# lorenlugosch/end-to-end-SLU

Measured on AMD Instinct MI355X. Metric: utterances/sec (train step, 3 s @16 kHz, B=64), higher is better.
Workload: dtype f32 (trainable stages: exact fp32 MFMA; convolutions and GRU contractions of FROZEN stages: bf16x3 = every fp32 operand split EXACTLY into 3 bf16 terms (3 x 8 = 24 significand bits, fp32's exponent range), 6 bf16 MFMA products per fp32 product (only terms below 2^-24 |a b| dropped), fp32 accumulatio; 1 GPU; experiments/no_unfreezing.cfg SLU train step (frozen SincNet/conv/biGRU encoder in train mode + intent biGRU trained): fwd + 3-slot CE + bwd + grad all-reduce + Adam; batch_per_gpu=64, global_batch=64, samples_per_utterance=48000, parallelism=dp1, encoder_lookahead_batches=20

## Files before the change

end-to-end-slu_amd/csrc/slu_api.hip:

```cpp
#include "slu_common.h"
#include <string.h>

namespace slu {
static thread_local char g_err[512] = "";
void set_error(const char* fmt, ...) {
  va_list ap;
  va_start(ap, fmt);
  vsnprintf(g_err, sizeof(g_err), fmt, ap);
  va_end(ap);
}
}

extern "C" int slu_version(void) { return SLU_ABI_VERSION; }

extern "C" const char* slu_last_error(void) { return slu::g_err; }

extern "C" const char* slu_device_arch(void) {
  static thread_local char arch[256];
  arch[0] = 0;
  int dev = 0;
  hipDeviceProp_t prop;
  if (hipGetDevice(&dev) != hipSuccess) return arch;
  if (hipGetDeviceProperties(&prop, dev) != hipSuccess) return arch;
  strncpy(arch, prop.gcnArchName, sizeof(arch) - 1);
  arch[sizeof(arch) - 1] = 0;
  return arch;
}

extern "C" int slu_device_check(void) {
  const char* a = slu_device_arch();
  if (strncmp(a, "gfx950", 6) != 0)
    SLU_FAIL(SLU_ERR_DEVICE, "libslu_hip is built for gfx950 (MI355X) only; current device is '%s'", a);
  return SLU_OK;
}

extern "C" int slu_stream_create_cu_range(int64_t first_cu, int64_t n_cus, void** stream_out) {
  SLU_REQUIRE(stream_out, "slu_stream_create_cu_range: null pointer");
  int dev = 0;
  hipDeviceProp_t prop;
  if (hipGetDevice(&dev) != hipSuccess || hipGetDeviceProperties(&prop, dev) != hipSuccess)
    SLU_FAIL(SLU_ERR_DEVICE, "slu_stream_create_cu_range: no HIP device");
  const int64_t total = prop.multiProcessorCount;
  SLU_REQUIRE(first_cu >= 0 && n_cus > 0 && first_cu + n_cus <= total,
              "slu_stream_create_cu_range: range [%lld, %lld) outside the %lld CUs of the device",
              (long long)first_cu, (long long)(first_cu + n_cus), (long long)total);
  uint32_t mask[32] = {0};
  SLU_REQUIRE(total <= 32 * 32, "slu_stream_create_cu_range: device too large");
  for (int64_t i = first_cu; i < first_cu + n_cus; ++i) mask[i >> 5] |= 1u << (i & 31);
  hipStream_t st = nullptr;
  const hipError_t e = hipExtStreamCreateWithCUMask(&st, (uint32_t)((total + 31) / 32), mask);
  if (e != hipSuccess) SLU_FAIL(SLU_ERR_HIP, "hipExtStreamCreateWithCUMask: %s", hipGetErrorString(e));
  *stream_out = (void*)st;
  return SLU_OK;
}

namespace slu {
struct StageSeg { const unsigned char* src; unsigned char* dst; long long rows, row_bytes, src_stride; };
struct StageArgs { StageSeg seg[4]; int nseg; long long* set_ptr; long long set_value; };

__global__ void __launch_bounds__(256)
stage_inputs_kernel(const StageArgs a) {
  if (blockIdx.x == 0 && threadIdx.x == 0 && a.set_ptr) *a.set_ptr = a.set_value;
  for (int k = 0; k < a.nseg; ++k) {
    const StageSeg sg = a.seg[k];
    const bool vec = ((sg.row_bytes | sg.src_stride | (long long)(uintptr_t)sg.src | (long long)(uintptr_t)sg.dst) & 15) == 0;
    if (vec) {
      const long long per_row = sg.row_bytes >> 4, total = sg.rows * per_row;
      for (long long i = (long long)blockIdx.x * 256 + threadIdx.x; i < total; i += (long long)gridDim.x * 256) {
        const long long r = i / per_row, c = i - r * per_row;
        reinterpret_cast<uint4*>(sg.dst + r * sg.row_bytes)[c] = reinterpret_cast<const uint4*>(sg.src + r * sg.src_stride)[c];
      }
    } else {
      const long long total = sg.rows * sg.row_bytes;
      for (long long i = (long long)blockIdx.x * 256 + threadIdx.x; i < total; i += (long long)gridDim.x * 256) {
        const long long r = i / sg.row_bytes, c = i - r * sg.row_bytes;
        sg.dst[r * sg.row_bytes + c] = sg.src[r * sg.src_stride + c];
      }
    }
  }
}
}

namespace slu {
struct StoreArgs { unsigned long long v[64]; unsigned long long* dst; int n; };
__global__ void store_u64_kernel(const StoreArgs a) {
  if ((int)threadIdx.x < a.n) a.dst[threadIdx.x] = a.v[threadIdx.x];
}
}

extern "C" int slu_store_u64(uint64_t* dst, const uint64_t* values, int64_t count, void* stream) {
  SLU_REQUIRE(dst && values && count >= 1 && count <= 64, "slu_store_u64: 1..64 values");
  slu::StoreArgs a;
  for (int k = 0; k < (int)count; ++k) a.v[k] = values[k];
  a.dst = (unsigned long long*)dst; a.n = (int)count;
  hipLaunchKernelGGL(slu::store_u64_kernel, dim3(1), dim3(64), 0, (hipStream_t)stream, a);
  SLU_CHECK_LAUNCH("store_u64_kernel");
  return SLU_OK;
}

extern "C" int slu_stage_inputs(const void* const* src, void* const* dst, const int64_t* rows, const int64_t* row_bytes,
                                const int64_t* src_stride_bytes, int64_t count, int64_t* set_ptr, int64_t set_value,
                                void* stream) {
  SLU_REQUIRE(count >= 0 && count <= 4, "slu_stage_inputs: at most 4 segments");
  slu::StageArgs a;
  long long bytes = 0;
  for (int k = 0; k < (int)count; ++k) {
    SLU_REQUIRE(src[k] && dst[k] && rows[k] > 0 && row_bytes[k] > 0, "slu_stage_inputs: bad segment %d", k);
    a.seg[k].src = (const unsigned char*)src[k]; a.seg[k].dst = (unsigned char*)dst[k];
    a.seg[k].rows = rows[k]; a.seg[k].row_bytes = row_bytes[k]; a.seg[k].src_stride = src_stride_bytes[k];
    bytes += rows[k] * row_bytes[k];
  }
  a.nseg = (int)count; a.set_ptr = (long long*)set_ptr; a.set_value = set_value;
  long long blocks = (bytes / 16 + 255) / 256;
  if (blocks < 1) blocks = 1;
  if (blocks > 512) blocks = 512;
  hipLaunchKernelGGL(slu::stage_inputs_kernel, dim3((unsigned)blocks), dim3(256), 0, (hipStream_t)stream, a);
  SLU_CHECK_LAUNCH("stage_inputs_kernel");
  return SLU_OK;
}

namespace slu {
constexpr int MULTI_MAX = 32;
struct MultiArgs { const unsigned char* src[MULTI_MAX]; unsigned char* dst[MULTI_MAX]; long long bytes[MULTI_MAX]; int n; };

__global__ void __launch_bounds__(256)
copy_multi_kernel(const MultiArgs a) {
  const int k = blockIdx.y;
  if (k >= a.n) return;
  const unsigned char* __restrict__ s = a.src[k];
  unsigned char* __restrict__ d = a.dst[k];
  const long long nb = a.bytes[k];
  const bool vec = (((long long)(uintptr_t)s | (long long)(uintptr_t)d | nb) & 15) == 0;
  if (vec) {
    for (long long i = (long long)blockIdx.x * 256 + threadIdx.x; i < (nb >> 4); i += (long long)gridDim.x * 256)
      reinterpret_cast<uint4*>(d)[i] = reinterpret_cast<const uint4*>(s)[i];
  } else {
    for (long long i = (long long)blockIdx.x * 256 + threadIdx.x; i < (nb >> 2); i += (long long)gridDim.x * 256)
      reinterpret_cast<unsigned*>(d)[i] = reinterpret_cast<const unsigned*>(s)[i];
  }
}

struct ScaleArgs { float* ptr[MULTI_MAX]; long long numel[MULTI_MAX]; int n; const float* g; };

__global__ void __launch_bounds__(256)
scale_multi_kernel(const ScaleArgs a) {
  const int k = blockIdx.y;
  if (k >= a.n) return;
  const float g = a.g[0];
  float* __restrict__ p = a.ptr[k];
  for (long long i = (long long)blockIdx.x * 256 + threadIdx.x; i < a.numel[k]; i += (long long)gridDim.x * 256) p[i] *= g;
}
}

extern "C" int slu_multi_max(void) { return slu::MULTI_MAX; }

extern "C" int slu_copy_multi(const void* const* src, void* const* dst, const int64_t* nbytes, int64_t count, void* stream) {
  SLU_REQUIRE(src && dst && nbytes && count >= 1 && count <= slu::MULTI_MAX, "slu_copy_multi: 1..%d segments", slu::MULTI_MAX);
  slu::MultiArgs a;
  long long most = 0;
  for (int k = 0; k < (int)count; ++k) {
    SLU_REQUIRE(src[k] && dst[k] && nbytes[k] > 0 && nbytes[k] % 4 == 0 && (((uintptr_t)src[k] | (uintptr_t)dst[k]) & 3) == 0,
                "slu_copy_multi: segment %d must be a non-empty, 4-byte aligned run of whole words", k);
    a.src[k] = (const unsigned char*)src[k]; a.dst[k] = (unsigned char*)dst[k]; a.bytes[k] = nbytes[k];
    if (nbytes[k] > most) most = nbytes[k];
  }
  a.n = (int)count;
  long long bx = (most / 16 + 255) / 256;
  if (bx < 1) bx = 1;
  if (bx > 64) bx = 64;
  hipLaunchKernelGGL(slu::copy_multi_kernel, dim3((unsigned)bx, (unsigned)count), dim3(256), 0, (hipStream_t)stream, a);
  SLU_CHECK_LAUNCH("copy_multi_kernel");
  return SLU_OK;
}

extern "C" int slu_scale_multi(float* const* ptrs, const int64_t* numel, int64_t count, const float* scale_dev, void* stream) {
  SLU_REQUIRE(ptrs && numel && scale_dev && count >= 1 && count <= slu::MULTI_MAX, "slu_scale_multi: 1..%d tensors", slu::MULTI_MAX);
  slu::ScaleArgs a;
  long long most = 0;
  for (int k = 0; k < (int)count; ++k) {
    SLU_REQUIRE(ptrs[k] && numel[k] > 0, "slu_scale_multi: bad tensor %d", k);
    a.ptr[k] = ptrs[k]; a.numel[k] = numel[k];
    if (numel[k] > most) most = numel[k];
  }
  a.n = (int)count; a.g = scale_dev;
  long long bx = (most + 1023) / 1024;
  if (bx < 1) bx = 1;
  if (bx > 256) bx = 256;
  hipLaunchKernelGGL(slu::scale_multi_kernel, dim3((unsigned)bx, (unsigned)count), dim3(256), 0, (hipStream_t)stream, a);
  SLU_CHECK_LAUNCH("scale_multi_kernel");
  return SLU_OK;
}

namespace slu {
struct AbsmaxArgs { const float* ptr[MULTI_MAX]; long long numel[MULTI_MAX]; int n; unsigned* words; };

__global__ void __launch_bounds__(256)
absmax_multi_kernel(const AbsmaxArgs a) {
  const int k = blockIdx.y;
  if (k >= a.n) return;
  const float* __restrict__ p = a.ptr[k];
  unsigned mx = 0;
  for (long long i = (long long)blockIdx.x * 256 + threadIdx.x; i < a.numel[k]; i += (long long)gridDim.x * 256)
    mx = max(mx, __float_as_uint(p[i]) & 0x7fffffffu);
#pragma unroll
  for (int d = 32; d >= 1; d >>= 1) mx = max(mx, (unsigned)__shfl_xor((int)mx, d, 64));
  if ((threadIdx.x & 63) == 0 && mx > 0) atomicMax(a.words + k, mx);
// ... 37 lines not shown
```

end-to-end-slu_amd/csrc/slu_common.h:

```cpp
#pragma once
#include <hip/hip_runtime.h>
#include <stdint.h>
#include <stdio.h>
#include <stdarg.h>
#include "../../include/slu_hip.h"

namespace slu {

void set_error(const char* fmt, ...);

#define SLU_FAIL(code, ...)            \
  do {                                 \
    ::slu::set_error(__VA_ARGS__);     \
    return (code);                     \
  } while (0)

#define SLU_REQUIRE(cond, ...)                          \
  do {                                                  \
    if (!(cond)) SLU_FAIL(SLU_ERR_INVALID_ARG, __VA_ARGS__); \
  } while (0)

#define SLU_CHECK_LAUNCH(name)                                                        \
  do {                                                                                \
    hipError_t e__ = hipGetLastError();                                               \
    if (e__ != hipSuccess) SLU_FAIL(SLU_ERR_HIP, "%s: %s", name, hipGetErrorString(e__)); \
  } while (0)

static inline int64_t cdiv(int64_t a, int64_t b) { return (a + b - 1) / b; }

typedef float f32x4 __attribute__((ext_vector_type(4)));

__device__ __forceinline__ f32x4 mfma16(float a, float b, f32x4 c) {
  return __builtin_amdgcn_mfma_f32_16x16x4f32(a, b, c, 0, 0, 0);
}

__device__ __forceinline__ float sigmoidf_acc(float x) { return 1.0f / (1.0f + expf(-x)); }

}
```

end-to-end-slu_amd/csrc/slu_gemm_bf16.hip:

```cpp
#include "slu_bf16.h"

#include <cstdlib>

namespace slu {

constexpr int GB_BM = 128, GB_BN = 64, GB_THREADS = 256;

struct GemmBfParams {
  const unsigned short* A;
  long long a_plane, lda;
  const uint4* wp;
  const float* bias;
  float* C; long long ldc;
  int M, N, KC;
};

template <int NS>
__global__ void __launch_bounds__(256)
gemm_bf_pack_kernel(const float* __restrict__ W, long long ldw, long long w_cs, uint4* __restrict__ wp, int N, int K, int KC, int NT) {
  const int idx = blockIdx.x * blockDim.x + threadIdx.x;
  if (idx >= KC * NT * 64) return;
  const int lane = idx & 63, nt = (idx >> 6) % NT, kc = (idx >> 6) / NT;
  const int n = nt * 16 + (lane & 15), k0 = kc * 32 + (lane >> 4) * 8;
  unsigned short h[NS][8];
// ... 107 lines not shown
    const int kn = min((kc_) + 1, p.KC - 1);                                                         \
               \
    uint4 fa[NS][4];                                                                                 \
    _Pragma("unroll") for (int pl = 0; pl < NS; ++pl) _Pragma("unroll") for (int a = 0; a < 4; ++a)  \
      fa[pl][a] = sA[buf * STAGE_U4 + pl * GB_BM * 4 + a_frag[a]];                                   \
    __builtin_amdgcn_sched_barrier(0);                                                               \
    GB_DMA_A(kn, 1 - buf) GB_FETCH_B(kn, nxt)                                                        \
    __builtin_amdgcn_sched_barrier(0);             \
    _Pragma("unroll") for (int q = 0; q < SP::NPAIR; ++q) {                                          \
      _Pragma("unroll") for (int a = 0; a < 4; ++a) _Pragma("unroll") for (int b = 0; b < 2; ++b)    \
        accs[SP::ACC(q)][a][b] = mfma_split<NS>(fa[SP::PA(q)][a], cur[SP::PB(q)][b], accs[SP::ACC(q)][a][b]); \
    }                                                                                                \
    __builtin_amdgcn_sched_barrier(0);        \
    __syncthreads();              \
  }
  GB_DMA_A(0, 0)
  GB_FETCH_B(0, rb0)
  __syncthreads();
  for (int kc = 0; kc < p.KC; kc += 2) {
    GB_STEP(kc, 0, rb0, rb1)
    if (kc + 1 < p.KC) GB_STEP(kc + 1, 1, rb1, rb0)
  }
#undef GB_STEP
#undef GB_FETCH_B
#undef GB_DMA_A
  f32x4 acc[4][2];
#pragma unroll
  for (int a = 0; a < 4; ++a)
#pragma unroll
    for (int b = 0; b < 2; ++b) acc[a][b] = split_result<NS>(accs[0][a][b], accs[SP::NACC - 1][a][b]);

  float* const sC = reinterpret_cast<float*>(smem) + wave * (32 * 36);
  const int col4 = (lane & 7) * 4;
  float4 bv = make_float4(0.f, 0.f, 0.f, 0.f);
  const int ncol = n0 + wn * 32 + col4;
  if (p.bias) { bv.x = p.bias[ncol]; bv.y = p.bias[ncol + 1]; bv.z = p.bias[ncol + 2]; bv.w = p.bias[ncol + 3]; }
#pragma unroll
  for (int h = 0; h < 2; ++h) {
#pragma unroll
    for (int a2 = 0; a2 < 2; ++a2)
#pragma unroll
      for (int b = 0; b < 2; ++b)
#pragma unroll
        for (int r = 0; r < 4; ++r) sC[(a2 * 16 + 4 * kg + r) * 36 + b * 16 + i] = acc[2 * h + a2][b][r];
#pragma unroll
    for (int it = 0; it < 4; ++it) {
      const int rl = (lane >> 3) + 8 * it;
      const int m = m0 + wm * 64 + h * 32 + rl;
      const float4 v = *reinterpret_cast<const float4*>(&sC[rl * 36 + col4]);
      if (m < p.M)
        *reinterpret_cast<float4*>(p.C + (size_t)m * p.ldc + ncol) = make_float4(v.x + bv.x, v.y + bv.y, v.z + bv.z, v.w + bv.w);
    }
  }
}


template <int NS, int KC>
__global__ void __launch_bounds__(GB_THREADS, 2)
gemm_bf_panel_kernel(const GemmBfParams p) {
  constexpr int STAGE_U4 = NS * GB_BM * 4;
  constexpr int EPI_FLOATS = 4 * 32 * 36;
  __shared__ __attribute__((aligned(16))) char smem[KC * STAGE_U4 * 16 + EPI_FLOATS * 4];
  uint4* const sA = reinterpret_cast<uint4*>(smem);
  const int tid = threadIdx.x, lane = tid & 63;
  const int wave = __builtin_amdgcn_readfirstlane(tid >> 6);
  const int wm = wave >> 1, wn = wave & 1;
  const int i = lane & 15, kg = lane >> 4;
  const int NT = p.N / 16, NJ = p.N / GB_BN;
  const int m0 = blockIdx.x * GB_BM;
  typedef const __attribute__((address_space(1))) void* gptr_t;
  typedef __attribute__((address_space(3))) void* lptr_t;
  {
    const int srow = tid >> 2, sslot = tid & 3;
#pragma unroll
    for (int h = 0; h < 2; ++h) {
      const int r = srow + 64 * h, m = m0 + r;
      const unsigned short* src = p.A + (size_t)(m < p.M ? m : 0) * p.lda + swz_slot(r, sslot) * 8;
#pragma unroll
      for (int kc = 0; kc < KC; ++kc)
#pragma unroll
        for (int pl = 0; pl < NS; ++pl)
          __builtin_amdgcn_global_load_lds((gptr_t)(src + (size_t)pl * p.a_plane + kc * 32),
                                           (lptr_t)(sA + kc * STAGE_U4 + (pl * GB_BM + 64 * h + 16 * wave) * 4), 16, 0, 0);
    }
  }
  const uint4* b_src = p.wp + (size_t)(wn * 2) * 64 + lane;
  const size_t b_plane = (size_t)p.KC * NT * 64, b_chunk = (size_t)NT * 64;
  int a_frag[4];
#pragma unroll
  for (int a = 0; a < 4; ++a) {
    const int r = wm * 64 + a * 16 + i;
    a_frag[a] = r * 4 + swz_slot(r, kg);
  }
  const int col4 = (lane & 7) * 4;
  float* const sC = reinterpret_cast<float*>(smem + KC * STAGE_U4 * 16) + wave * (32 * 36);
  typedef Split<NS> SP;
  uint4 rb0[KC][NS][2], rb1[KC][NS][2];
  float4 bias0 = make_float4(0.f, 0.f, 0.f, 0.f), bias1 = bias0;
#define GP_FETCH(j_, dst, bdst)                                                                         \
  {                                                                                                     \
    const int jj = min((j_), NJ - 1);                                                                   \
    _Pragma("unroll") for (int kc = 0; kc < KC; ++kc) _Pragma("unroll") for (int pl = 0; pl < NS; ++pl) \
      _Pragma("unroll") for (int b = 0; b < 2; ++b)                                                     \
        dst[kc][pl][b] = b_src[(size_t)pl * b_plane + (size_t)kc * b_chunk + (size_t)(jj * 4 + b) * 64]; \
    if (p.bias) bdst = *reinterpret_cast<const float4*>(p.bias + jj * GB_BN + wn * 32 + col4);          \
  }
#define GP_TILE(j_, cur, bcur, nxt, bnxt)                                                               \
  {                                                                                                     \
    GP_FETCH((j_) + 1, nxt, bnxt)                                                                       \
    __builtin_amdgcn_sched_barrier(0);    \
    f32x4 accs[SP::NACC][4][2];                                                                         \
    _Pragma("unroll") for (int c = 0; c < SP::NACC; ++c)                                                \
      _Pragma("unroll") for (int a = 0; a < 4; ++a) _Pragma("unroll") for (int b = 0; b < 2; ++b)       \
        accs[c][a][b] = f32x4{0.f, 0.f, 0.f, 0.f};                                                      \
    _Pragma("unroll") for (int kc = 0; kc < KC; ++kc) {                                                 \
      uint4 fa[NS][4];                                                                                  \
      _Pragma("unroll") for (int pl = 0; pl < NS; ++pl) _Pragma("unroll") for (int a = 0; a < 4; ++a)   \
        fa[pl][a] = sA[kc * STAGE_U4 + pl * GB_BM * 4 + a_frag[a]];                                     \
      _Pragma("unroll") for (int q = 0; q < SP::NPAIR; ++q) {                                           \
        _Pragma("unroll") for (int a = 0; a < 4; ++a) _Pragma("unroll") for (int b = 0; b < 2; ++b)     \
          accs[SP::ACC(q)][a][b] = mfma_split<NS>(fa[SP::PA(q)][a], cur[kc][SP::PB(q)][b], accs[SP::ACC(q)][a][b]); \
      }                                                                                                 \
    }                                                                                                   \
    f32x4 acc[4][2];                                                                                    \
    _Pragma("unroll") for (int a = 0; a < 4; ++a) _Pragma("unroll") for (int b = 0; b < 2; ++b)         \
      acc[a][b] = split_result<NS>(accs[0][a][b], accs[SP::NACC - 1][a][b]);                            \
    const int ncol = (j_) * GB_BN + wn * 32 + col4;                                                     \
    _Pragma("unroll") for (int h = 0; h < 2; ++h) {                                                     \
      _Pragma("unroll") for (int a2 = 0; a2 < 2; ++a2) _Pragma("unroll") for (int b = 0; b < 2; ++b)    \
        _Pragma("unroll") for (int r = 0; r < 4; ++r)                                                   \
          sC[(a2 * 16 + 4 * kg + r) * 36 + b * 16 + i] = acc[2 * h + a2][b][r];                         \
      _Pragma("unroll") for (int it = 0; it < 4; ++it) {                                                \
        const int rl = (lane >> 3) + 8 * it;                                                            \
        const int m = m0 + wm * 64 + h * 32 + rl;                                                       \
        const float4 v = *reinterpret_cast<const float4*>(&sC[rl * 36 + col4]);                         \
        if (m < p.M)                                                                                    \
          *reinterpret_cast<float4*>(p.C + (size_t)m * p.ldc + ncol) =                                  \
              make_float4(v.x + bcur.x, v.y + bcur.y, v.z + bcur.z, v.w + bcur.w);                      \
      }                                                                                                 \
    }                                                                                                   \
  }
  GP_FETCH(0, rb0, bias0)
  __syncthreads();
  for (int j = 0; j < NJ; j += 2) {
    GP_TILE(j, rb0, bias0, rb1, bias1)
    if (j + 1 < NJ) GP_TILE(j + 1, rb1, bias1, rb0, bias0)
  }
#undef GP_TILE
#undef GP_FETCH
}


constexpr int GP_ROWS = 96;
constexpr int64_t GP_PANEL_MIN_M = 16 * 1024;

template <int NS, int KC>
__global__ void __launch_bounds__(GB_THREADS, 1)
gemm_bf_panel96_kernel(const GemmBfParams p) {
  constexpr int CH_U4 = NS * GP_ROWS * 4;
  typedef Split<NS> SP;
  extern __shared__ __attribute__((aligned(16))) char dsmem[];
  uint4* const sA = reinterpret_cast<uint4*>(dsmem);
  const int tid = threadIdx.x, lane = tid & 63;
  const int wave = __builtin_amdgcn_readfirstlane(tid >> 6);
  const int wm = wave >> 1, wn = wave & 1;
  const int i = lane & 15, kg = lane >> 4;
  const int NT = p.N / 16, NJ = p.N / GB_BN;
  const int m0 = blockIdx.x * GP_ROWS;
  typedef const __attribute__((address_space(1))) void* gptr_t;
  typedef __attribute__((address_space(3))) void* lptr_t;
  {
    const int rrow = lane >> 2, rslot = lane & 3;
    for (int u = wave; u < KC * NS * (GP_ROWS / 16); u += 4) {
      const int rg = u % (GP_ROWS / 16), pl = (u / (GP_ROWS / 16)) % NS, kc = u / ((GP_ROWS / 16) * NS);
      const int r = rg * 16 + rrow, m = m0 + r;
      const unsigned short* src = p.A + (size_t)pl * p.a_plane + (size_t)(m < p.M ? m : 0) * p.lda + kc * 32 + swz_slot(r, rslot) * 8;
      __builtin_amdgcn_global_load_lds((gptr_t)src, (lptr_t)(sA + kc * CH_U4 + (pl * GP_ROWS + rg * 16) * 4), 16, 0, 0);
    }
  }
  const uint4* b_src = p.wp + (size_t)(wn * 2) * 64 + lane;
  const size_t b_plane = (size_t)p.KC * NT * 64, b_chunk = (size_t)NT * 64;
  int a_frag[3];
#pragma unroll
  for (int a = 0; a < 3; ++a) {
    const int r = wm * 48 + a * 16 + i;
    a_frag[a] = r * 4 + swz_slot(r, kg);
  }
  const int col4 = (lane & 7) * 4;
  float* const sC = reinterpret_cast<float*>(dsmem + (size_t)KC * CH_U4 * 16) + wave * (16 * 36);

  uint4 wr[4][NS][2];
#define G9_FETCH(s_, set_)                                                                              \
  {                                                                                                     \
    const int ss = min((s_), NJ * KC - 1);                                                              \
    const int jj = ss / KC, kk = ss - jj * KC;                                                          \
    _Pragma("unroll") for (int pl = 0; pl < NS; ++pl) _Pragma("unroll") for (int b = 0; b < 2; ++b)     \
      wr[set_][pl][b] = b_src[(size_t)pl * b_plane + (size_t)kk * b_chunk + (size_t)(jj * 4 + b) * 64]; \
  }
  G9_FETCH(0, 0) G9_FETCH(1, 1) G9_FETCH(2, 2)
  __syncthreads();

  f32x4 accs[SP::NACC][3][2];
  float4 bias_v = make_float4(0.f, 0.f, 0.f, 0.f);
#define G9_READ_A(s_, dst)                                                                              \
  {                                                                                                     \
    const int kc_ = (s_) % KC;                                                                          \
    _Pragma("unroll") for (int pl = 0; pl < NS; ++pl) _Pragma("unroll") for (int a = 0; a < 3; ++a)     \
      dst[pl][a] = sA[kc_ * CH_U4 + pl * GP_ROWS * 4 + a_frag[a]];                                      \
  }
#ifndef SLU_G9_SCHED
#define SLU_G9_SCHED 1
#endif
#define G9_STEP(s_, SET, fcur, fnxt)                                                                    \
  {                                                                                                     \
    G9_FETCH((s_) + 3, (SET + 3) % 4)                                                                   \
    G9_READ_A((s_) + 1, fnxt)                                                                           \
    if constexpr (SLU_G9_SCHED == 0) __builtin_amdgcn_sched_barrier(0);                                 \
    _Pragma("unroll") for (int q = 0; q < SP::NPAIR; ++q) {                                             \
      _Pragma("unroll") for (int a = 0; a < 3; ++a) _Pragma("unroll") for (int b = 0; b < 2; ++b)       \
        accs[SP::ACC(q)][a][b] = mfma_split<NS>(fcur[SP::PA(q)][a], wr[SET][SP::PB(q)][b], accs[SP::ACC(q)][a][b]); \
    }                                                                                                   \
    if constexpr (SLU_G9_SCHED == 0) {                                                                  \
      __builtin_amdgcn_sched_barrier(0);                                                                \
    } else {                                                                                            \
                                                                                \
      _Pragma("unroll") for (int g_ = 0; g_ < 2 * NS; ++g_) {                                           \
        __builtin_amdgcn_sched_group_barrier(0x008, 1, 0);                                              \
        __builtin_amdgcn_sched_group_barrier(0x020, 1, 0);                                              \
      }                                                                                                 \
      _Pragma("unroll") for (int g_ = 0; g_ < 3 * NS; ++g_) {                                           \
        __builtin_amdgcn_sched_group_barrier(0x008, 1, 0);                                              \
        __builtin_amdgcn_sched_group_barrier(0x100, 1, 0);                                              \
      }                                                                                                 \
      __builtin_amdgcn_sched_group_barrier(0x008, SP::NPAIR * 6 - 5 * NS, 0);                           \
    }                                                                                                   \
  }
  uint4 fa0[NS][3], fa1[NS][3];
  G9_READ_A(0, fa0)
  static_assert(KC % 4 == 0, "the register ring assumes a multiple of four k-chunks per tile");
  for (int j = 0; j < NJ; ++j) {
#pragma unroll
    for (int c = 0; c < SP::NACC; ++c)
#pragma unroll
      for (int a = 0; a < 3; ++a) { accs[c][a][0] = f32x4{0.f, 0.f, 0.f, 0.f}; accs[c][a][1] = f32x4{0.f, 0.f, 0.f, 0.f}; }
    if (p.bias) bias_v = *reinterpret_cast<const float4*>(p.bias + j * GB_BN + wn * 32 + col4);
#pragma unroll
    for (int k4 = 0; k4 < KC; k4 += 4) {
      G9_STEP(j * KC + k4 + 0, 0, fa0, fa1)
      G9_STEP(j * KC + k4 + 1, 1, fa1, fa0)
      G9_STEP(j * KC + k4 + 2, 2, fa0, fa1)
      G9_STEP(j * KC + k4 + 3, 3, fa1, fa0)
    }
    f32x4 acc[3][2];
#pragma unroll
    for (int a = 0; a < 3; ++a)
#pragma unroll
      for (int b = 0; b < 2; ++b) acc[a][b] = split_result<NS>(accs[0][a][b], accs[SP::NACC - 1][a][b]);
    const int ncol = j * GB_BN + wn * 32 + col4;
#pragma unroll
    for (int a = 0; a < 3; ++a) {
#pragma unroll
      for (int b = 0; b < 2; ++b)
#pragma unroll
        for (int r = 0; r < 4; ++r) sC[(4 * kg + r) * 36 + b * 16 + i] = acc[a][b][r];
#pragma unroll
      for (int it = 0; it < 2; ++it) {
        const int rl = (lane >> 3) + 8 * it;
        const int m = m0 + wm * 48 + a * 16 + rl;
        const float4 v = *reinterpret_cast<const float4*>(&sC[rl * 36 + col4]);
        if (m < p.M)
          *reinterpret_cast<float4*>(p.C + (size_t)m * p.ldc + ncol) =
              make_float4(v.x + bias_v.x, v.y + bias_v.y, v.z + bias_v.z, v.w + bias_v.w);
      }
    }
  }
#undef G9_STEP
#undef G9_READ_A
#undef G9_FETCH
}


template <int NS>
__global__ void __launch_bounds__(GB_THREADS, 2)
gemm_bf_a32_kernel(const float* __restrict__ A32, long long lda32, int K, const GemmBfParams p) {
  constexpr int STAGE_U4 = NS * GB_BM * 4;
  constexpr int EPI_FLOATS = 4 * 32 * 36;
  constexpr int SMEM_BYTES = (2 * STAGE_U4 * 16 > EPI_FLOATS * 4) ? 2 * STAGE_U4 * 16 : EPI_FLOATS * 4;
  __shared__ __attribute__((aligned(16))) char smem[SMEM_BYTES];
  uint4* const sA = reinterpret_cast<uint4*>(smem);
  typedef Split<NS> SP;
  const int tid = threadIdx.x, lane = tid & 63;
  const int wave = __builtin_amdgcn_readfirstlane(tid >> 6);
  const int wm = wave >> 1, wn = wave & 1;
  const int i = lane & 15, kg = lane >> 4;
  const int NT = (p.N + 15) / 16;
  int bx = blockIdx.x, by = blockIdx.y;
  {
    const int total = gridDim.x * gridDim.y;
    const int L = blockIdx.y * gridDim.x + blockIdx.x;
    if ((total & 7) == 0) {
      const int V = (L & 7) * (total >> 3) + (L >> 3);
      by = V / gridDim.x;
      bx = V - by * gridDim.x;
    }
  }
  const int m0 = by * GB_BM, n0 = bx * GB_BN;

  f32x4 accs[SP::NACC][4][2];
#pragma unroll
  for (int c = 0; c < SP::NACC; ++c)
#pragma unroll
    for (int a = 0; a < 4; ++a)
#pragma unroll
      for (int b = 0; b < 2; ++b) accs[c][a][b] = f32x4{0.f, 0.f, 0.f, 0.f};

  const int srow = tid >> 1, shalf = tid & 1;
  const float* __restrict__ arow = A32 + (size_t)(m0 + srow < p.M ? m0 + srow : 0) * lda32;
  const int s_slot0 = srow * 4 + swz_slot(srow, 2 * shalf), s_slot1 = srow * 4 + swz_slot(srow, 2 * shalf + 1);
  float4 pre[4];
#define GA_LOAD(kc_)                                                                         \
  _Pragma("unroll") for (int v = 0; v < 4; ++v) {                                            \
    const int k = (kc_) * 32 + shalf * 16 + v * 4;                                           \
    pre[v] = *reinterpret_cast<const float4*>(arow + (k < K ? k : 0));    \
  }
#define GA_STORE(buf_, kc_)                                                                  \
  {                                                                                          \
    unsigned short h[16][NS];                                                                \
    _Pragma("unroll") for (int v = 0; v < 4; ++v) {                                          \
      if ((kc_) * 32 + shalf * 16 + v * 4 >= K) pre[v] = make_float4(0.f, 0.f, 0.f, 0.f);    \
      split_terms<NS>(pre[v].x, h[4 * v]); split_terms<NS>(pre[v].y, h[4 * v + 1]);          \
      split_terms<NS>(pre[v].z, h[4 * v + 2]); split_terms<NS>(pre[v].w, h[4 * v + 3]);      \
    }                                                                                        \
    _Pragma("unroll") for (int pl = 0; pl < NS; ++pl) {                                      \
      uint4 o0, o1;                                                                          \
      o0.x = h[0][pl] | ((unsigned)h[1][pl] << 16);   o0.y = h[2][pl] | ((unsigned)h[3][pl] << 16);   \
      o0.z = h[4][pl] | ((unsigned)h[5][pl] << 16);   o0.w = h[6][pl] | ((unsigned)h[7][pl] << 16);   \
      o1.x = h[8][pl] | ((unsigned)h[9][pl] << 16);   o1.y = h[10][pl] | ((unsigned)h[11][pl] << 16); \
      o1.z = h[12][pl] | ((unsigned)h[13][pl] << 16); o1.w = h[14][pl] | ((unsigned)h[15][pl] << 16); \
      sA[(buf_) * STAGE_U4 + pl * GB_BM * 4 + s_slot0] = o0;                                 \
      sA[(buf_) * STAGE_U4 + pl * GB_BM * 4 + s_slot1] = o1;                                 \
    }                                                                                        \
  }
  const uint4* b_src = p.wp + lane;
  const int b_tile[2] = {min(n0 / 16 + wn * 2, NT - 1) * 64, min(n0 / 16 + wn * 2 + 1, NT - 1) * 64};
  const size_t b_plane = (size_t)p.KC * NT * 64, b_chunk = (size_t)NT * 64;
  int a_frag[4];
#pragma unroll
  for (int a = 0; a < 4; ++a) {
    const int r = wm * 64 + a * 16 + i;
    a_frag[a] = r * 4 + swz_slot(r, kg);
  }
  uint4 rb0[NS][2], rb1[NS][2];
#define GA_FETCH_B(kc_, dst)                                                                         \
  _Pragma("unroll") for (int pl = 0; pl < NS; ++pl) _Pragma("unroll") for (int b = 0; b < 2; ++b)    \
    dst[pl][b] = b_src[(size_t)pl * b_plane + (size_t)(kc_) * b_chunk + b_tile[b]];
#define GA_STEP(kc_, buf, cur, nxt)                              \
  {                                                                                                  \
    const int kn = min((kc_) + 1, p.KC - 1);                                                         \
    uint4 fa[NS][4];                                                                                 \
    _Pragma("unroll") for (int pl = 0; pl < NS; ++pl) _Pragma("unroll") for (int a = 0; a < 4; ++a)  \
      fa[pl][a] = sA[buf * STAGE_U4 + pl * GB_BM * 4 + a_frag[a]];                                   \
    GA_FETCH_B(kn, nxt)                                                                              \
    __builtin_amdgcn_sched_barrier(0);                                                               \
    _Pragma("unroll") for (int q = 0; q < SP::NPAIR; ++q) {                                          \
      _Pragma("unroll") for (int a = 0; a < 4; ++a) _Pragma("unroll") for (int b = 0; b < 2; ++b)    \
        accs[SP::ACC(q)][a][b] = mfma_split<NS>(fa[SP::PA(q)][a], cur[SP::PB(q)][b], accs[SP::ACC(q)][a][b]); \
    }                                                                                                \
    __builtin_amdgcn_sched_barrier(0);                                                               \
    if ((kc_) + 1 < p.KC) {           \
      GA_STORE(1 - buf, (kc_) + 1)                                                                   \
      if ((kc_) + 2 < p.KC) { GA_LOAD((kc_) + 2) }                                                   \
    }                                                                                                \
    __syncthreads();                                                                                 \
  }
  GA_LOAD(0)
  GA_FETCH_B(0, rb0)
  GA_STORE(0, 0)
  if (p.KC > 1) { GA_LOAD(1) }
  __syncthreads();
  for (int kc = 0; kc < p.KC; kc += 2) {
    GA_STEP(kc, 0, rb0, rb1)
    if (kc + 1 < p.KC) GA_STEP(kc + 1, 1, rb1, rb0)
  }
#undef GA_STEP
#undef GA_FETCH_B
#undef GA_STORE
#undef GA_LOAD
  f32x4 acc[4][2];
#pragma unroll
  for (int a = 0; a < 4; ++a)
#pragma unroll
    for (int b = 0; b < 2; ++b) acc[a][b] = split_result<NS>(accs[0][a][b], accs[SP::NACC - 1][a][b]);

  float* const sC = reinterpret_cast<float*>(smem) + wave * (32 * 36);
  const int col4 = (lane & 7) * 4;
  float4 bv = make_float4(0.f, 0.f, 0.f, 0.f);
  const int ncol = n0 + wn * 32 + col4;
  const bool col_ok = ncol < p.N;
  if (p.bias && col_ok) { bv.x = p.bias[ncol]; bv.y = p.bias[ncol + 1]; bv.z = p.bias[ncol + 2]; bv.w = p.bias[ncol + 3]; }
#pragma unroll
  for (int h = 0; h < 2; ++h) {
#pragma unroll
    for (int a2 = 0; a2 < 2; ++a2)
#pragma unroll
      for (int b = 0; b < 2; ++b)
#pragma unroll
        for (int r = 0; r < 4; ++r) sC[(a2 * 16 + 4 * kg + r) * 36 + b * 16 + i] = acc[2 * h + a2][b][r];
#pragma unroll
    for (int it = 0; it < 4; ++it) {
      const int rl = (lane >> 3) + 8 * it;
      const int m = m0 + wm * 64 + h * 32 + rl;
      const float4 v = *reinterpret_cast<const float4*>(&sC[rl * 36 + col4]);
      if (m < p.M && col_ok)
        *reinterpret_cast<float4*>(p.C + (size_t)m * p.ldc + ncol) = make_float4(v.x + bv.x, v.y + bv.y, v.z + bv.z, v.w + bv.w);
    }
  }
}

}

using namespace slu;

extern "C" size_t slu_gemm_bf16_pack_bytes(int64_t N, int64_t K, int nsplit) {
  return (size_t)nsplit * cdiv(K, 32) * cdiv(N, 16) * 64 * sizeof(uint4);
}

extern "C" int slu_gemm_bf16_pack(const float* W, int64_t ldw, int64_t w_cs, void* packed, int64_t N, int64_t K, int nsplit,
                                  void* stream) {
  SLU_REQUIRE(W && packed && N > 0 && K > 0, "slu_gemm_bf16_pack: bad argument");
  SLU_REQUIRE(nsplit >= 1 && nsplit <= 3, "slu_gemm_bf16_pack: nsplit must be 1 (bf16), 2 (f16x2) or 3 (bf16x3)");
  const int KC = (int)cdiv(K, 32), NT = (int)cdiv(N, 16);
  const int total = KC * NT * 64;
#define SLU_PACK(NS_) hipLaunchKernelGGL(gemm_bf_pack_kernel<NS_>, dim3((total + 255) / 256), dim3(256), 0, (hipStream_t)stream, W, \
                                         (long long)ldw, (long long)w_cs, (uint4*)packed, (int)N, (int)K, KC, NT)
  if (nsplit == 3) SLU_PACK(3); else if (nsplit == 2) SLU_PACK(2); else SLU_PACK(1);
#undef SLU_PACK
  SLU_CHECK_LAUNCH("gemm_bf_pack_kernel");
  return SLU_OK;
}

extern "C" int slu_split_bf16(const float* x, int64_t ldx, void* planes, int64_t plane_stride, int64_t rows,
                              int64_t K, int nsplit, void* stream) {
  SLU_REQUIRE(x && planes && rows > 0 && K > 0, "slu_split_bf16: bad argument");
  SLU_REQUIRE(nsplit >= 1 && nsplit <= 3, "slu_split_bf16: nsplit must be 1 (bf16), 2 (f16x2) or 3 (bf16x3)");
  const int Kp = (int)(cdiv(K, 32) * 32);
  SLU_REQUIRE(plane_stride >= rows * Kp, "slu_split_bf16: plane stride smaller than rows * round_up(K, 32)");
  const long long total = rows * (Kp / 8);
#define SLU_SPLIT(NS_) hipLaunchKernelGGL(split_planes_kernel<NS_>, dim3((unsigned)cdiv(total, 256)), dim3(256), 0, (hipStream_t)stream, x, \
                                          (long long)ldx, (unsigned short*)planes, (long long)plane_stride, (long long)rows, (int)K, Kp)
  if (nsplit == 3) SLU_SPLIT(3); else if (nsplit == 2) SLU_SPLIT(2); else SLU_SPLIT(1);
#undef SLU_SPLIT
  SLU_CHECK_LAUNCH("split_planes_kernel");
  return SLU_OK;
}

extern "C" int slu_gemm_bf16(const void* A_planes, int64_t a_plane_stride, int64_t lda, const void* w_packed,
                             const float* bias, float* C, int64_t ldc, int64_t M, int64_t N, int64_t K,
                             int nsplit, void* stream) {
  SLU_REQUIRE(A_planes && w_packed && C, "slu_gemm_bf16: null pointer");
  SLU_REQUIRE(M > 0 && N > 0 && K > 0, "slu_gemm_bf16: non-positive size");
  SLU_REQUIRE(nsplit >= 1 && nsplit <= 3, "slu_gemm_bf16: nsplit must be 1 (bf16), 2 (f16x2) or 3 (bf16x3)");
  if (N % GB_BN != 0) SLU_FAIL(SLU_ERR_UNSUPPORTED, "slu_gemm_bf16: N = %lld is not a multiple of %d", (long long)N, GB_BN);
  const int64_t Kp = cdiv(K, 32) * 32;
  SLU_REQUIRE(lda >= Kp && (lda % 8) == 0, "slu_gemm_bf16: lda must be >= round_up(K, 32) and a multiple of 8");
  SLU_REQUIRE((ldc % 4) == 0, "slu_gemm_bf16: ldc must be a multiple of 4");
  GemmBfParams p;
  p.A = (const unsigned short*)A_planes; p.a_plane = a_plane_stride; p.lda = lda;
  p.wp = (const uint4*)w_packed; p.bias = bias; p.C = C; p.ldc = ldc;
  p.M = (int)M; p.N = (int)N; p.KC = (int)(Kp / 32);
  if (p.KC <= 2 && N >= 2 * GB_BN && (bias == nullptr || ((uintptr_t)bias & 15) == 0)) {
    const dim3 pg((unsigned)cdiv(M, GB_BM));
    hipStream_t st = (hipStream_t)stream;
#define SLU_PANEL(NS_)                                                                                    \
    { if (p.KC == 2) hipLaunchKernelGGL((gemm_bf_panel_kernel<NS_, 2>), pg, dim3(GB_THREADS), 0, st, p); \
      else hipLaunchKernelGGL((gemm_bf_panel_kernel<NS_, 1>), pg, dim3(GB_THREADS), 0, st, p); }
    if (nsplit == 3) SLU_PANEL(3) else if (nsplit == 2) SLU_PANEL(2) else SLU_PANEL(1)
#undef SLU_PANEL
    SLU_CHECK_LAUNCH("gemm_bf_panel_kernel");
    return SLU_OK;
  }
  if ((p.KC == 4 || p.KC == 8) && N >= 2 * GB_BN && M >= GP_PANEL_MIN_M && (bias == nullptr || ((uintptr_t)bias & 15) == 0)
      && !(getenv("SLU_GEMM_PANEL96") && atoi(getenv("SLU_GEMM_PANEL96")) == 0)) {
    const size_t lds = (size_t)p.KC * nsplit * GP_ROWS * 64 + 4 * 16 * 36 * sizeof(float);
    const dim3 pg((unsigned)cdiv(M, GP_ROWS));
    hipStream_t st = (hipStream_t)stream;
#define SLU_P96(NS_, KC_)                                                                                            \
    {                                                                                                                \
      hipError_t e = hipFuncSetAttribute((const void*)gemm_bf_panel96_kernel<NS_, KC_>,                              \
                                         hipFuncAttributeMaxDynamicSharedMemorySize, (int)lds);                      \
      if (e != hipSuccess) SLU_FAIL(SLU_ERR_HIP, "slu_gemm_bf16: cannot raise the dynamic LDS cap to %zu: %s", lds, hipGetErrorString(e)); \
      hipLaunchKernelGGL((gemm_bf_panel96_kernel<NS_, KC_>), pg, dim3(GB_THREADS), lds, st, p);                      \
    }
    if (nsplit == 3 && p.KC == 8) SLU_P96(3, 8)
    else if (nsplit == 3) SLU_P96(3, 4)
    else if (nsplit == 2 && p.KC == 8) SLU_P96(2, 8)
    else if (nsplit == 2) SLU_P96(2, 4)
    else if (p.KC == 8) SLU_P96(1, 8)
    else SLU_P96(1, 4)
#undef SLU_P96
    SLU_CHECK_LAUNCH("gemm_bf_panel96_kernel");
    return SLU_OK;
  }
  dim3 grid((unsigned)(N / GB_BN), (unsigned)cdiv(M, GB_BM));
  SLU_REQUIRE(grid.y <= 65535, "slu_gemm_bf16: M too large for one launch");
  if (nsplit == 3) hipLaunchKernelGGL(gemm_bf_kernel<3>, grid, dim3(GB_THREADS), 0, (hipStream_t)stream, p);
  else if (nsplit == 2) hipLaunchKernelGGL(gemm_bf_kernel<2>, grid, dim3(GB_THREADS), 0, (hipStream_t)stream, p);
  else hipLaunchKernelGGL(gemm_bf_kernel<1>, grid, dim3(GB_THREADS), 0, (hipStream_t)stream, p);
  SLU_CHECK_LAUNCH("gemm_bf_kernel");
  return SLU_OK;
}

extern "C" int slu_gemm_bf16_a32(const float* A, int64_t lda, const void* w_packed, const float* bias, float* C, int64_t ldc,
                                 int64_t M, int64_t N, int64_t K, int nsplit, void* stream) {
  SLU_REQUIRE(A && w_packed && C, "slu_gemm_bf16_a32: null pointer");
  SLU_REQUIRE(M > 0 && N > 0 && K > 0, "slu_gemm_bf16_a32: non-positive size");
  SLU_REQUIRE(nsplit >= 1 && nsplit <= 3, "slu_gemm_bf16_a32: nsplit must be 1 (bf16), 2 (f16x2) or 3 (bf16x3)");
  if ((N & 3) || (K & 3) || (lda & 3) || (ldc & 3) || ((uintptr_t)A & 15) || ((uintptr_t)C & 15) || lda < K)
    SLU_FAIL(SLU_ERR_UNSUPPORTED, "slu_gemm_bf16_a32: needs N, K, lda, ldc multiples of 4 and 16-byte aligned A, C "
             "(N %lld, K %lld, lda %lld, ldc %lld)", (long long)N, (long long)K, (long long)lda, (long long)ldc);
  GemmBfParams p;
  p.A = nullptr; p.a_plane = 0; p.lda = 0;
  p.wp = (const uint4*)w_packed; p.bias = bias; p.C = C; p.ldc = ldc;
  p.M = (int)M; p.N = (int)N; p.KC = (int)cdiv(K, 32);
  dim3 grid((unsigned)cdiv(N, GB_BN), (unsigned)cdiv(M, GB_BM));
  SLU_REQUIRE(grid.y <= 65535, "slu_gemm_bf16_a32: M too large for one launch");
  hipStream_t st = (hipStream_t)stream;
  if (nsplit == 3) hipLaunchKernelGGL(gemm_bf_a32_kernel<3>, grid, dim3(GB_THREADS), 0, st, A, (long long)lda, (int)K, p);
  else if (nsplit == 2) hipLaunchKernelGGL(gemm_bf_a32_kernel<2>, grid, dim3(GB_THREADS), 0, st, A, (long long)lda, (int)K, p);
  else hipLaunchKernelGGL(gemm_bf_a32_kernel<1>, grid, dim3(GB_THREADS), 0, st, A, (long long)lda, (int)K, p);
  SLU_CHECK_LAUNCH("gemm_bf_a32_kernel");
  return SLU_OK;
}

namespace slu {

constexpr int TNB_T = 64;
constexpr int TNB_K = 32;
constexpr int TNB_LD = 40;

struct TnBfParams {
  const float* A; long long lda;
  const float* B; long long ldb;
  float* out; long long ldc;
  long long slab;
  int M, N, K, k_per_split;
};

template <int NS>
__device__ __forceinline__ void tnb_stage(unsigned short* __restrict__ s, const float4& v0, const float4& v1, int c4, int kp) {
  const float e0[4] = {v0.x, v0.y, v0.z, v0.w}, e1[4] = {v1.x, v1.y, v1.z, v1.w};
#pragma unroll
  for (int j = 0; j < 4; ++j) {
    unsigned short h0[NS], h1[NS];
    split_terms<NS>(e0[j], h0);
    split_terms<NS>(e1[j], h1);
#pragma unroll
    for (int pl = 0; pl < NS; ++pl)
      *reinterpret_cast<unsigned*>(s + pl * (TNB_T * TNB_LD) + (c4 + j) * TNB_LD + kp) = h0[pl] | ((unsigned)h1[pl] << 16);
  }
}

template <int NS>
__global__ void __launch_bounds__(256)
gemm_tn_bf16_kernel(const TnBfParams p) {
  typedef Split<NS> SP;
  __shared__ __attribute__((aligned(16))) unsigned short sA[2][NS * TNB_T * TNB_LD];
  __shared__ __attribute__((aligned(16))) unsigned short sB[2][NS * TNB_T * TNB_LD];
  const int tid = threadIdx.x, lane = tid & 63, w = tid >> 6;
  const int m0 = blockIdx.y * TNB_T, n0 = blockIdx.x * TNB_T;
  const int k_begin = blockIdx.z * p.k_per_split;
  const int k_end = min(p.K, k_begin + p.k_per_split);
  const int kp = (tid >> 4) * 2, c4 = (tid & 15) * 4;
  const bool a_in = m0 + c4 < p.M, b_in = n0 + c4 < p.N;
  const float* __restrict__ Ap = p.A + (a_in ? m0 + c4 : 0);
  const float* __restrict__ Bp = p.B + (b_in ? n0 + c4 : 0);
  const float4 zero = make_float4(0.f, 0.f, 0.f, 0.f);

  auto load = [&](int k0, float4& a0, float4& a1, float4& b0, float4& b1) {
    const int ka = k0 + kp, kb = k0 + kp + 1;
    a0 = (a_in && ka < k_end) ? *reinterpret_cast<const float4*>(Ap + (long long)ka * p.lda) : zero;
    a1 = (a_in && kb < k_end) ? *reinterpret_cast<const float4*>(Ap + (long long)kb * p.lda) : zero;
    b0 = (b_in && ka < k_end) ? *reinterpret_cast<const float4*>(Bp + (long long)ka * p.ldb) : zero;
    b1 = (b_in && kb < k_end) ? *reinterpret_cast<const float4*>(Bp + (long long)kb * p.ldb) : zero;
  };

  float4 a0, a1, b0, b1;
  load(k_begin, a0, a1, b0, b1);
  tnb_stage<NS>(sA[0], a0, a1, c4, kp);
  tnb_stage<NS>(sB[0], b0, b1, c4, kp);
  __syncthreads();

  const int wm = w >> 1, wn = w & 1;
  const int i = lane & 15, kg = lane >> 4;
  f32x4 accs[SP::NACC][2][2];
#pragma unroll
  for (int c = 0; c < SP::NACC; ++c)
#pragma unroll
    for (int mt = 0; mt < 2; ++mt)
#pragma unroll
      for (int nt = 0; nt < 2; ++nt) accs[c][mt][nt] = f32x4{0.f, 0.f, 0.f, 0.f};

  int buf = 0;
  for (int k0 = k_begin; k0 < k_end; k0 += TNB_K) {
    const bool more = k0 + TNB_K < k_end;
    if (more) load(k0 + TNB_K, a0, a1, b0, b1);
    uint4 fa[NS][2], fb[NS][2];
#pragma unroll
    for (int pl = 0; pl < NS; ++pl) {
#pragma unroll
      for (int mt = 0; mt < 2; ++mt)
        fa[pl][mt] = *reinterpret_cast<const uint4*>(&sA[buf][pl * (TNB_T * TNB_LD) + (wm * 32 + mt * 16 + i) * TNB_LD + kg * 8]);
#pragma unroll
      for (int nt = 0; nt < 2; ++nt)
        fb[pl][nt] = *reinterpret_cast<const uint4*>(&sB[buf][pl * (TNB_T * TNB_LD) + (wn * 32 + nt * 16 + i) * TNB_LD + kg * 8]);
    }
#pragma unroll
    for (int q = 0; q < SP::NPAIR; ++q)
#pragma unroll
      for (int mt = 0; mt < 2; ++mt)
#pragma unroll
        for (int nt = 0; nt < 2; ++nt)
          accs[SP::ACC(q)][mt][nt] = mfma_split<NS>(fa[SP::PA(q)][mt], fb[SP::PB(q)][nt], accs[SP::ACC(q)][mt][nt]);
    if (more) {
      tnb_stage<NS>(sA[buf ^ 1], a0, a1, c4, kp);
      tnb_stage<NS>(sB[buf ^ 1], b0, b1, c4, kp);
    }
    __syncthreads();
    buf ^= 1;
  }

  float* __restrict__ out = p.out + (size_t)blockIdx.z * p.slab;
#pragma unroll
  for (int mt = 0; mt < 2; ++mt)
#pragma unroll
    for (int nt = 0; nt < 2; ++nt) {
      const f32x4 acc = split_result<NS>(accs[0][mt][nt], accs[SP::NACC - 1][mt][nt]);
#pragma unroll
      for (int r = 0; r < 4; ++r) {
        const int m = m0 + wm * 32 + mt * 16 + 4 * kg + r, n = n0 + wn * 32 + nt * 16 + i;
        if (m < p.M && n < p.N) out[(size_t)m * p.ldc + n] = acc[r];
      }
    }
}

// ... 66 lines not shown
```

Baseline: 377,000 utterances/s.

## Make panel96 GEMM persistent per CU and split tail panels across column blocks

The panel96 bf16 GEMM now launches one block per CU of the stream's CU mask, not one per 96-row panel. Each block loops over panels in rounds. When the last partial round is at most half the CUs, those panels are split along the N column-block range so the tail wave keeps more CUs busy. A registry of CU-masked streams lets the host learn the CU count for each stream. In exchange, tail blocks reload the A panel redundantly, there is an extra sync between panels, and the host does a mutex lookup on every launch.

```diff
diff --git a/end-to-end-slu_amd/csrc/slu_api.hip b/end-to-end-slu_amd/csrc/slu_api.hip
--- a/end-to-end-slu_amd/csrc/slu_api.hip
+++ b/end-to-end-slu_amd/csrc/slu_api.hip
@@ -1,8 +1,14 @@
 #include "slu_common.h"
 #include <string.h>
+#include <mutex>
+#include <utility>
+#include <vector>
 
 namespace slu {
 static thread_local char g_err[512] = "";
+static std::mutex g_cu_mu;
+static std::vector<std::pair<hipStream_t, int>> g_cu_streams;
+static int g_dev_cus[64] = {0};
 void set_error(const char* fmt, ...) {
   va_list ap;
   va_start(ap, fmt);
@@ -50,8 +56,26 @@
   hipStream_t st = nullptr;
   const hipError_t e = hipExtStreamCreateWithCUMask(&st, (uint32_t)((total + 31) / 32), mask);
   if (e != hipSuccess) SLU_FAIL(SLU_ERR_HIP, "hipExtStreamCreateWithCUMask: %s", hipGetErrorString(e));
+  {
+    std::lock_guard<std::mutex> lock(slu::g_cu_mu);
+    slu::g_cu_streams.emplace_back(st, (int)n_cus);
+  }
   *stream_out = (void*)st;
   return SLU_OK;
+}
+
+int slu::stream_cus(hipStream_t stream) {
+  std::lock_guard<std::mutex> lock(g_cu_mu);
+  for (const auto& s : g_cu_streams)
+    if (s.first == stream) return s.second;
+  int dev = 0;
+  if (hipGetDevice(&dev) != hipSuccess || dev < 0 || dev >= 64) return 0;
+  if (g_dev_cus[dev] == 0) {
+    int n = 0;
+    if (hipDeviceGetAttribute(&n, hipDeviceAttributeMultiprocessorCount, dev) != hipSuccess) return 0;
+    g_dev_cus[dev] = n;
+  }
+  return g_dev_cus[dev];
 }
 
 namespace slu {
diff --git a/end-to-end-slu_amd/csrc/slu_common.h b/end-to-end-slu_amd/csrc/slu_common.h
--- a/end-to-end-slu_amd/csrc/slu_common.h
+++ b/end-to-end-slu_amd/csrc/slu_common.h
@@ -8,6 +8,8 @@
 namespace slu {
 
 void set_error(const char* fmt, ...);
+
+int stream_cus(hipStream_t stream);
 
 #define SLU_FAIL(code, ...)            \
   do {                                 \
diff --git a/end-to-end-slu_amd/csrc/slu_gemm_bf16.hip b/end-to-end-slu_amd/csrc/slu_gemm_bf16.hip
--- a/end-to-end-slu_amd/csrc/slu_gemm_bf16.hip
+++ b/end-to-end-slu_amd/csrc/slu_gemm_bf16.hip
@@ -283,11 +283,21 @@
 
 
 constexpr int GP_ROWS = 96;
+struct Panel96Plan { int rounds, rem, split; };
+
+static inline unsigned panel96_plan(int64_t panels, int NJ, int cus, Panel96Plan* plan) {
+  const int64_t G = cus > 0 ? cus : 1;
+  plan->rounds = (int)(panels / G);
+  plan->rem = (int)(panels % G);
+  plan->split = 1;
+  if (plan->rem > 0 && 2 * (int64_t)plan->rem <= G) plan->split = (int)((G / plan->rem) < NJ ? (G / plan->rem) : NJ);
+  return (unsigned)(plan->rounds > 0 ? G : (int64_t)plan->rem * plan->split);
+}
 constexpr int64_t GP_PANEL_MIN_M = 16 * 1024;
 
 template <int NS, int KC>
 __global__ void __launch_bounds__(GB_THREADS, 1)
-gemm_bf_panel96_kernel(const GemmBfParams p) {
+gemm_bf_panel96_kernel(const GemmBfParams p, const Panel96Plan plan) {
   constexpr int CH_U4 = NS * GP_ROWS * 4;
   typedef Split<NS> SP;
   extern __shared__ __attribute__((aligned(16))) char dsmem[];
@@ -297,18 +307,8 @@
   const int wm = wave >> 1, wn = wave & 1;
   const int i = lane & 15, kg = lane >> 4;
   const int NT = p.N / 16, NJ = p.N / GB_BN;
-  const int m0 = blockIdx.x * GP_ROWS;
   typedef const __attribute__((address_space(1))) void* gptr_t;
   typedef __attribute__((address_space(3))) void* lptr_t;
-  {
-    const int rrow = lane >> 2, rslot = lane & 3;
-    for (int u = wave; u < KC * NS * (GP_ROWS / 16); u += 4) {
-      const int rg = u % (GP_ROWS / 16), pl = (u / (GP_ROWS / 16)) % NS, kc = u / ((GP_ROWS / 16) * NS);
-      const int r = rg * 16 + rrow, m = m0 + r;
-      const unsigned short* src = p.A + (size_t)pl * p.a_plane + (size_t)(m < p.M ? m : 0) * p.lda + kc * 32 + swz_slot(r, rslot) * 8;
-      __builtin_amdgcn_global_load_lds((gptr_t)src, (lptr_t)(sA + kc * CH_U4 + (pl * GP_ROWS + rg * 16) * 4), 16, 0, 0);
-    }
-  }
   const uint4* b_src = p.wp + (size_t)(wn * 2) * 64 + lane;
   const size_t b_plane = (size_t)p.KC * NT * 64, b_chunk = (size_t)NT * 64;
   int a_frag[3];
@@ -323,13 +323,11 @@
   uint4 wr[4][NS][2];
 #define G9_FETCH(s_, set_)                                                                              \
   {                                                                                                     \
-    const int ss = min((s_), NJ * KC - 1);                                                              \
-    const int jj = ss / KC, kk = ss - jj * KC;                                                          \
+    const int ss = min((s_), (j1 - j0) * KC - 1);                                                       \
+    const int jj = j0 + ss / KC, kk = ss % KC;                                                          \
     _Pragma("unroll") for (int pl = 0; pl < NS; ++pl) _Pragma("unroll") for (int b = 0; b < 2; ++b)     \
       wr[set_][pl][b] = b_src[(size_t)pl * b_plane + (size_t)kk * b_chunk + (size_t)(jj * 4 + b) * 64]; \
   }
-  G9_FETCH(0, 0) G9_FETCH(1, 1) G9_FETCH(2, 2)
-  __syncthreads();
 
   f32x4 accs[SP::NACC][3][2];
   float4 bias_v = make_float4(0.f, 0.f, 0.f, 0.f);
@@ -367,9 +365,32 @@
     }                                                                                                   \
   }
   uint4 fa0[NS][3], fa1[NS][3];
+  static_assert(KC % 4 == 0, "the register ring assumes a multiple of four k-chunks per tile");
+  const int G = gridDim.x, w = blockIdx.x;
+  const int visits = plan.rounds + (w < plan.rem * plan.split ? 1 : 0);
+  for (int vis = 0; vis < visits; ++vis) {
+  int panel = vis * G + w, j0 = 0, j1 = NJ;
+  if (vis >= plan.rounds) {
+    const int q = w / plan.rem;
+    panel = plan.rounds * G + w % plan.rem;
+    j0 = q * NJ / plan.split;
+    j1 = (q + 1) * NJ / plan.split;
+  }
+  const int m0 = panel * GP_ROWS;
+  if (vis > 0) __syncthreads();
+  {
+    const int rrow = lane >> 2, rslot = lane & 3;
+    for (int u = wave; u < KC * NS * (GP_ROWS / 16); u += 4) {
+      const int rg = u % (GP_ROWS / 16), pl = (u / (GP_ROWS / 16)) % NS, kc = u / ((GP_ROWS / 16) * NS);
+      const int r = rg * 16 + rrow, m = m0 + r;
+      const unsigned short* src = p.A + (size_t)pl * p.a_plane + (size_t)(m < p.M ? m : 0) * p.lda + kc * 32 + swz_slot(r, rslot) * 8;
+      __builtin_amdgcn_global_load_lds((gptr_t)src, (lptr_t)(sA + kc * CH_U4 + (pl * GP_ROWS + rg * 16) * 4), 16, 0, 0);
+    }
+  }
+  G9_FETCH(0, 0) G9_FETCH(1, 1) G9_FETCH(2, 2)
+  __syncthreads();
   G9_READ_A(0, fa0)
-  static_assert(KC % 4 == 0, "the register ring assumes a multiple of four k-chunks per tile");
-  for (int j = 0; j < NJ; ++j) {
+  for (int j = j0; j < j1; ++j) {
 #pragma unroll
     for (int c = 0; c < SP::NACC; ++c)
 #pragma unroll
@@ -377,10 +398,10 @@
     if (p.bias) bias_v = *reinterpret_cast<const float4*>(p.bias + j * GB_BN + wn * 32 + col4);
 #pragma unroll
     for (int k4 = 0; k4 < KC; k4 += 4) {
-      G9_STEP(j * KC + k4 + 0, 0, fa0, fa1)
-      G9_STEP(j * KC + k4 + 1, 1, fa1, fa0)
-      G9_STEP(j * KC + k4 + 2, 2, fa0, fa1)
-      G9_STEP(j * KC + k4 + 3, 3, fa1, fa0)
+      G9_STEP((j - j0) * KC + k4 + 0, 0, fa0, fa1)
+      G9_STEP((j - j0) * KC + k4 + 1, 1, fa1, fa0)
+      G9_STEP((j - j0) * KC + k4 + 2, 2, fa0, fa1)
+      G9_STEP((j - j0) * KC + k4 + 3, 3, fa1, fa0)
     }
     f32x4 acc[3][2];
 #pragma unroll
@@ -404,6 +425,7 @@
               make_float4(v.x + bias_v.x, v.y + bias_v.y, v.z + bias_v.z, v.w + bias_v.w);
       }
     }
+  }
   }
 #undef G9_STEP
 #undef G9_READ_A
@@ -613,14 +635,16 @@
   if ((p.KC == 4 || p.KC == 8) && N >= 2 * GB_BN && M >= GP_PANEL_MIN_M && (bias == nullptr || ((uintptr_t)bias & 15) == 0)
       && !(getenv("SLU_GEMM_PANEL96") && atoi(getenv("SLU_GEMM_PANEL96")) == 0)) {
     const size_t lds = (size_t)p.KC * nsplit * GP_ROWS * 64 + 4 * 16 * 36 * sizeof(float);
-    const dim3 pg((unsigned)cdiv(M, GP_ROWS));
     hipStream_t st = (hipStream_t)stream;
-#define SLU_P96(NS_, KC_)                                                                                            \
+    Panel96Plan plan;
+    SLU_REQUIRE(stream_cus(st) > 0, "slu_gemm_bf16: cannot learn the CU count of the device");
+    const dim3 pg(panel96_plan(cdiv(M, GP_ROWS), (int)(N / GB_BN), stream_cus(st), &plan));
+#define SLU_P96(NS_, KC_)                                                                                           \
     {                                                                                                                \
       hipError_t e = hipFuncSetAttribute((const void*)gemm_bf_panel96_kernel<NS_, KC_>,                              \
                                          hipFuncAttributeMaxDynamicSharedMemorySize, (int)lds);                      \
       if (e != hipSuccess) SLU_FAIL(SLU_ERR_HIP, "slu_gemm_bf16: cannot raise the dynamic LDS cap to %zu: %s", lds, hipGetErrorString(e)); \
-      hipLaunchKernelGGL((gemm_bf_panel96_kernel<NS_, KC_>), pg, dim3(GB_THREADS), lds, st, p);                      \
+      hipLaunchKernelGGL((gemm_bf_panel96_kernel<NS_, KC_>), pg, dim3(GB_THREADS), lds, st, p, plan);                \
     }
     if (nsplit == 3 && p.KC == 8) SLU_P96(3, 8)
     else if (nsplit == 3) SLU_P96(3, 4)
```

New measurement: 382,300 utterances/s (median of 6 runs). +1.4%, better.
